# jdfxzzy/DPMN

Measured on AMD Instinct MI355X. Metric: SR images/sec (16x64->32x128, bs=48 per GPU, fp32 forward), higher is better.
Workload: dtype f32; 1 GPU; cfg1: TATT PSN + 3+3 PGRM (embed 96, windows 2/4/8) + CMM, forward-only; per_gpu_batch=48, global_batch=48, ranks=1, batches_in_flight=2, parallelism=dp1 (independent batch shards, no forward collective)

## Files before the change

dpmn_amd/csrc/common.h:

```cpp
#pragma once
#include <hip/hip_runtime.h>
#include <stdint.h>
#include "../../include/dpmn_hip.h"

typedef float f32x4 __attribute__((ext_vector_type(4)));

#define DPMN_CHECK_LAUNCH()                                                         \
  do {                                                                              \
    hipError_t e__ = hipGetLastError();                                             \
    if (e__ != hipSuccess) return dpmn_set_error(DPMN_ERR_LAUNCH, hipGetErrorString(e__)); \
  } while (0)

#define DPMN_REQUIRE(cond, msg)                                    \
  do {                                                             \
    if (!(cond)) return dpmn_set_error(DPMN_ERR_ARG, msg);         \
  } while (0)

int dpmn_set_error(int code, const char* msg);

__device__ __forceinline__ f32x4 mfma16(float a, float b, f32x4 c) {
  return __builtin_amdgcn_mfma_f32_16x16x4f32(a, b, c, 0, 0, 0);
}

__device__ __forceinline__ float erf_as(float x) {
// ... 97 lines not shown
    case 16: return xshfl<16>(v);
    case 32: return xshfl<32>(v);
    default: return __shfl_xor(v, o, 64);
  }
}
__device__ __forceinline__ float wave_sum(float v) {
#pragma unroll
  for (int o = 32; o > 0; o >>= 1) v += xshfl_v(v, o);
  return v;
}
__device__ __forceinline__ float wave_max(float v) {
#pragma unroll
  for (int o = 32; o > 0; o >>= 1) v = fmaxf(v, xshfl_v(v, o));
  return v;
}

constexpr unsigned long long DROP_PHI = 0x9E3779B97F4A7C15ull;
__device__ __forceinline__ unsigned long long drop_z0(unsigned long long seed, unsigned long long idx) { return idx * DROP_PHI + seed; }
__device__ __forceinline__ float drop_scale_z(unsigned long long z, float p, float inv_keep) {
  z ^= z >> 30; z *= 0xBF58476D1CE4E5B9ull;
  z ^= z >> 27; z *= 0x94D049BB133111EBull;
  z ^= z >> 31;
  const float u = (float)(unsigned)(z >> 40) * 5.9604644775390625e-8f;
  return u >= p ? inv_keep : 0.0f;
}
__device__ __forceinline__ float drop_scale(unsigned long long seed, unsigned long long idx, float p, float inv_keep) {
  return drop_scale_z(drop_z0(seed, idx), p, inv_keep);
}

static inline hipStream_t as_stream(dpmn_stream_t s) { return (hipStream_t)s; }

enum ProfTag { PT_CONV_IGEMM_128 = 0, PT_CONV_IGEMM_64, PT_CONV_IGEMM_NARROW, PT_CONV_SPLITK_REDUCE, PT_CONV_HALO, PT_CONV_HALO_C4,
               PT_GEMM_PW, PT_GEMM_WSTAT, PT_GEMM_KLOOP, PT_DWCONV_GELU, PT_WATTN8, PT_WATTN_SCALAR, PT_ATTN_FUSED, PT_BIGRU,
               PT_MHA32, PT_PATCH_EMBED, PT_SK_GATE, PT_TAIL, PT_DWPW_FUSED, PT_GEMM_WSTAT_LN, PT_CONV_IGEMM_SK, PT_ATTN_FUSED_BWD, PT_WATTN_BWD,
               PT_CONV_WGRAD, PT_GEMM_TN, PT_TN_REDUCE, PT_DWCONV_BWD, PT_WGRAD_UNPACK, PT_CONV_PACK, PT_AFFINE_ACT_BWD, PT_LN_BWD, PT_WATTN_MFMA32, PT_COUNT };
extern unsigned long long g_dpmn_prof_mask;
extern double g_dpmn_prof_hint_bytes;
extern int g_dpmn_bf16;
extern int g_dpmn_x3;
typedef __bf16 bf16x2 __attribute__((ext_vector_type(2)));
typedef __bf16 bf16x8 __attribute__((ext_vector_type(8)));
__device__ __forceinline__ uint2 pack_bf16x4(float a, float b, float c, float d) {
  typedef float f32x2_ __attribute__((ext_vector_type(2)));
  const bf16x2 lo = __builtin_convertvector((f32x2_){a, b}, bf16x2), hi = __builtin_convertvector((f32x2_){c, d}, bf16x2);
  return make_uint2(__builtin_bit_cast(unsigned, lo), __builtin_bit_cast(unsigned, hi));
}
__device__ __forceinline__ f32x4 mfma16_bf16(bf16x8 a, bf16x8 b, f32x4 c) {
  return __builtin_amdgcn_mfma_f32_16x16x32_bf16(a, b, c, 0, 0, 0);
}
__device__ __forceinline__ void x3_split2t(float a, float b, unsigned& h, unsigned& m, unsigned& l) {
  const unsigned ua = __float_as_uint(a), ub = __float_as_uint(b);
  h = __builtin_amdgcn_perm(ub, ua, 0x07060302u);
  const float ra = a - __uint_as_float(ua & 0xffff0000u), rb = b - __uint_as_float(ub & 0xffff0000u);
  const unsigned va = __float_as_uint(ra), vb = __float_as_uint(rb);
  m = __builtin_amdgcn_perm(vb, va, 0x07060302u);
  const float sa = ra - __uint_as_float(va & 0xffff0000u), sb = rb - __uint_as_float(vb & 0xffff0000u);
  l = __builtin_amdgcn_perm(__float_as_uint(sb), __float_as_uint(sa), 0x07060302u);
}
__device__ __forceinline__ void x3_split4t(const float4& v, uint2& h, uint2& m, uint2& l) {
  x3_split2t(v.x, v.y, h.x, m.x, l.x);
  x3_split2t(v.z, v.w, h.y, m.y, l.y);
}
struct ProfScope {
  int slot;
  hipStream_t st;
  ProfScope(int tag, hipStream_t s, double flops, double bytes);
  ~ProfScope();
// ... 15 lines not shown
```

dpmn_amd/csrc/pgrm.hip:

```cpp
#include "common.h"

namespace {

template <int C, int PATCH, bool FUSE>
__global__ __launch_bounds__(256) void k_patch_embed_ln(const float* __restrict__ img, int cin, const float* __restrict__ pf_w,
                                                         const float* __restrict__ pf_b, const float* __restrict__ pe_w,
                                                         const float* __restrict__ pe_b, const float* __restrict__ ln_w,
                                                         const float* __restrict__ ln_b, float* __restrict__ tok, int B,
                                                         int Hi, int Wi, float p_drop, unsigned long long seed) {
  constexpr int CQ = C / 4, KP = 3 * PATCH * PATCH;
  static_assert(!FUSE || PATCH == 2, "fused prior conv assumes 2x2 patches (one pixel per lane of the token quad)");
  __shared__ __attribute__((aligned(16))) float wt[KP * C];
  __shared__ float pfw[3 * 2 * 9 + 3];
  for (int i = threadIdx.x; i < KP * C; i += 256) wt[(i % KP) * C + i / KP] = pe_w[i];
  if (FUSE && threadIdx.x < 57) pfw[threadIdx.x] = threadIdx.x < 54 ? pf_w[threadIdx.x] : pf_b[threadIdx.x - 54];
  __syncthreads();
  const int Ht = Hi / PATCH, Wt = Wi / PATCH;
  const int lane = threadIdx.x & 63;
  long token = (long)blockIdx.x * 64 + (threadIdx.x >> 6) * 16 + (lane >> 2);
  const long ntok = (long)B * Ht * Wt;
  const bool valid = token < ntok;
  if (!valid) token = ntok - 1;
  const int part = lane & 3;
  const int b = token / (Ht * Wt), t = token % (Ht * Wt);
  const int th = t / Wt, tw = t % Wt;
  float in[KP];
  if (FUSE) {
    const int dy = part >> 1, dx = part & 1;
    const int y = th * 2 + dy, x = tw * 2 + dx;
    float a[3] = {pfw[54], pfw[55], pfw[56]};
#pragma unroll
    for (int ci = 0; ci < 2; ++ci)
#pragma unroll
      for (int ky = 0; ky < 3; ++ky) {
        const int yy = y + ky - 1;
#pragma unroll
        for (int kx = 0; kx < 3; ++kx) {
          const int xx = x + kx - 1;
          const bool inb = yy >= 0 && yy < Hi && xx >= 0 && xx < Wi;
          const float v = inb ? img[(((size_t)b * 2 + ci) * Hi + yy) * Wi + xx] : 0.f;
#pragma unroll
          for (int c = 0; c < 3; ++c) a[c] += pfw[((c * 2 + ci) * 3 + ky) * 3 + kx] * v;
        }
      }
    const int base = lane & ~3;
#pragma unroll
// ... 2 lines not shown
      for (int pix = 0; pix < 4; ++pix) in[c * 4 + pix] = __shfl(a[c], base + pix, 64);
  } else {
#pragma unroll
    for (int c = 0; c < 3; ++c)
#pragma unroll
      for (int dy = 0; dy < PATCH; ++dy)
#pragma unroll
        for (int dx = 0; dx < PATCH; ++dx)
          in[(c * PATCH + dy) * PATCH + dx] = img[(((size_t)b * cin + c) * Hi + th * PATCH + dy) * Wi + tw * PATCH + dx];
  }
  float o[CQ], s = 0.f;
#pragma unroll
  for (int i = 0; i < CQ; i += 4) {
    const float4 b4 = *reinterpret_cast<const float4*>(pe_b + part * CQ + i);
    o[i] = b4.x; o[i + 1] = b4.y; o[i + 2] = b4.z; o[i + 3] = b4.w;
  }
#pragma unroll
  for (int k = 0; k < KP; ++k) {
#pragma unroll
    for (int i = 0; i < CQ; i += 4) {
      const float4 w4 = *reinterpret_cast<const float4*>(wt + k * C + part * CQ + i);
      o[i] += w4.x * in[k]; o[i + 1] += w4.y * in[k]; o[i + 2] += w4.z * in[k]; o[i + 3] += w4.w * in[k];
    }
  }
#pragma unroll
  for (int i = 0; i < CQ; ++i) s += o[i];
  s += xshfl<1>(s); s += xshfl<2>(s);
  const float mean = s * (1.0f / C);
  float q = 0.f;
#pragma unroll
  for (int i = 0; i < CQ; ++i) { const float d = o[i] - mean; q += d * d; }
  q += xshfl<1>(q); q += xshfl<2>(q);
  const float rstd = 1.0f / sqrtf(q * (1.0f / C) + 1e-5f);
  if (!valid) return;
  float* dst = tok + (size_t)token * C + part * CQ;
  const float ik = p_drop > 0.f ? 1.0f / (1.0f - p_drop) : 1.f;
#pragma unroll
  for (int i = 0; i < CQ; i += 4) {
    const int c = part * CQ + i;
    float v[4] = {(o[i] - mean) * rstd * ln_w[c] + ln_b[c], (o[i + 1] - mean) * rstd * ln_w[c + 1] + ln_b[c + 1],
                  (o[i + 2] - mean) * rstd * ln_w[c + 2] + ln_b[c + 2], (o[i + 3] - mean) * rstd * ln_w[c + 3] + ln_b[c + 3]};
    if (p_drop > 0.f) {
      const unsigned long long z0 = drop_z0(seed, (unsigned long long)token * C + c);
#pragma unroll
      for (int r = 0; r < 4; ++r) v[r] *= drop_scale_z(z0 + (unsigned long long)r * DROP_PHI, p_drop, ik);
    }
    *reinterpret_cast<float4*>(dst + i) = make_float4(v[0], v[1], v[2], v[3]);
  }
}

template <int WS, int D, bool DROP>
__global__ __launch_bounds__(256) void k_window_attn(const float* __restrict__ q, const float* __restrict__ kv,
                                                      const float* __restrict__ bias_table, float* __restrict__ out, int B,
                                                      int H, int W, int C, int g, int shift, float p_drop,
                                                      unsigned long long seed) {
  constexpr int N = WS * WS;
  constexpr int CG = 2 * D;
  constexpr int QROWS = 64;
  constexpr int KROWS = 64;
  constexpr int LDR = CG + 4;
  constexpr int TBL = (2 * WS - 1) * (2 * WS - 1);
  extern __shared__ __attribute__((aligned(16))) float smem[];
  float* tbl = smem;
  float* base = smem + ((TBL * 2 + 3) & ~3);
  const int wave = threadIdx.x >> 6, lane = threadIdx.x & 63;
  const int slab_in_blk = wave >> 1, head = wave & 1;
  float* Qs = base + slab_in_blk * (QROWS + 2 * KROWS) * LDR;
  float* Ks = Qs + QROWS * LDR;
  float* Vs = Ks + KROWS * LDR;
  int* reg_s = reinterpret_cast<int*>(base + 2 * (QROWS + 2 * KROWS) * LDR) + slab_in_blk * KROWS;

  const int L = H * W;
  const int slabs_per_img = L / QROWS;
  const long slab = (long)blockIdx.x * 2 + slab_in_blk;
  const int b = slab / slabs_per_img;
  const int t0 = (slab % slabs_per_img) * QROWS;
  const int nWc = W / WS;
  const bool active = b < B;

  for (int i = threadIdx.x; i < TBL * 2; i += 256) tbl[i] = bias_table[i];
// ... 369 lines not shown
  constexpr int N = WS * WS, CG = 2 * D, LDR = CG + 4, TBL = (2 * WS - 1) * (2 * WS - 1), ROWS = WS == 16 ? 256 : 64, SETS = WS == 16 ? 1 : 2;
  const size_t smem = (size_t)(((TBL * 2 + 3) & ~3) + SETS * 2 * ROWS * LDR) * 4 + (size_t)SETS * ROWS * 4;
  static bool attr_set = false;
  if (!attr_set) {
    (void)hipFuncSetAttribute(reinterpret_cast<const void*>(&k_window_attn_mfma<WS, D, DROP>), hipFuncAttributeMaxDynamicSharedMemorySize, (int)smem);
    attr_set = true;
  }
  const long sets = (long)B * (H * W / ROWS);
  ProfScope prof(PT_WATTN_MFMA32, st, 4.0 * N * D * 2 * (double)B * H * W, 4.0 * 4 * CG * (double)B * H * W);
  hipLaunchKernelGGL((k_window_attn_mfma<WS, D, DROP>), dim3((unsigned)((sets + SETS - 1) / SETS)), dim3(WS == 16 ? 512 : 256), smem, st, q, kv, table,
                     out, B, H, W, C, g, shift, p_drop, seed);
  DPMN_CHECK_LAUNCH();
  return DPMN_OK;
}

template <int WS, int D, bool DROP>
int launch_window_attn(const float* q, const float* kv, const float* table, float* out, int B, int H, int W, int C, int g,
                       int shift, float p_drop, unsigned long long seed, hipStream_t st) {
  constexpr int N = WS * WS, CG = 2 * D, KROWS = 64, LDR = CG + 4, TBL = (2 * WS - 1) * (2 * WS - 1);
  const size_t smem = (size_t)(((TBL * 2 + 3) & ~3) + 2 * (64 + 2 * KROWS) * LDR) * 4 + 2 * KROWS * 4;
  static bool attr_set = false;
  if (!attr_set) {
    (void)hipFuncSetAttribute(reinterpret_cast<const void*>(&k_window_attn<WS, D, DROP>), hipFuncAttributeMaxDynamicSharedMemorySize, (int)smem);
    attr_set = true;
  }
  const long slabs = (long)B * (H * W / 64);
  ProfScope prof(PT_WATTN_SCALAR, st, 4.0 * N * D * 2 * (double)B * H * W, 4.0 * 4 * CG * (double)B * H * W);
  hipLaunchKernelGGL((k_window_attn<WS, D, DROP>), dim3((unsigned)((slabs + 1) / 2)), dim3(256), smem, st, q, kv, table, out, B, H, W,
                     C, g, shift, p_drop, seed);
  DPMN_CHECK_LAUNCH();
  return DPMN_OK;
}

__global__ void k_sk_gate(const float* __restrict__ partial, int parts_per_image, int L, const float* __restrict__ fc1_w,
                          const float* __restrict__ fc1_b, const float* __restrict__ fc2_w, const float* __restrict__ fc2_b,
                          float* __restrict__ attn_vec, int C, int G, int dmid) {
  extern __shared__ float sm[];
  float* S = sm;
  float* Z = sm + C;
  float* A = Z + dmid;
  const int b = blockIdx.x;
  for (int c = threadIdx.x; c < C; c += blockDim.x) {
    const float* pp = partial + (size_t)b * parts_per_image * C + c;
    float s0 = 0.f, s1 = 0.f, s2 = 0.f, s3 = 0.f;
    int p = 0;
    for (; p + 4 <= parts_per_image; p += 4) {
      s0 += pp[(size_t)p * C]; s1 += pp[(size_t)(p + 1) * C]; s2 += pp[(size_t)(p + 2) * C]; s3 += pp[(size_t)(p + 3) * C];
    }
    for (; p < parts_per_image; ++p) s0 += pp[(size_t)p * C];
    S[c] = ((s0 + s1) + (s2 + s3)) / (float)L;
  }
  __syncthreads();
  for (int j0 = 0; j0 < dmid; j0 += blockDim.x / 8) {
    const int j = j0 + threadIdx.x / 8, part = threadIdx.x & 7;
    float a = 0.f;
    if (j < dmid)
      for (int c = part; c < C; c += 8) a += fc1_w[j * C + c] * S[c];
    a += xshfl<1>(a); a += xshfl<2>(a); a += xshfl<4>(a);
    if (j < dmid && part == 0) Z[j] = gelu_erf(a + fc1_b[j]);
  }
  __syncthreads();
  for (int c = threadIdx.x; c < C; c += blockDim.x) {
    float a = fc2_b[c];
#pragma unroll 8
    for (int j = 0; j < dmid; ++j) a += fc2_w[c * dmid + j] * Z[j];
    A[c] = a;
  }
  __syncthreads();
  const int cg = C / G;
  for (int c = threadIdx.x; c < cg; c += blockDim.x) {
    float mx = -INFINITY;
    for (int g = 0; g < G; ++g) mx = fmaxf(mx, A[g * cg + c]);
    float den = 0.f;
    for (int g = 0; g < G; ++g) den += expf(A[g * cg + c] - mx);
    for (int g = 0; g < G; ++g) attn_vec[((size_t)b * G + g) * cg + c] = expf(A[g * cg + c] - mx) / den;
  }
}

template <bool R32>
__global__ __launch_bounds__(256) void k_dwconv_gelu(const float* __restrict__ y, const float* __restrict__ w,
                                                      const float* __restrict__ bias, float* __restrict__ g, int Ch, int r,
                                                      long planes, int apply_gelu, float* __restrict__ g2 = nullptr, int in_gelu = 0,
                                                      float p_drop = 0.f, unsigned long long seed = 0ull, int rb = 0) {
  const float inv_keep = p_drop > 0.f ? 1.0f / (1.0f - p_drop) : 1.0f;
  extern __shared__ __attribute__((aligned(16))) float sm[];
  const int wave = threadIdx.x >> 6, lane = threadIdx.x & 63;
  if (R32 || rb <= 0) rb = r;
  const int nb = r / rb;
  const long vplane = (long)blockIdx.x * 4 + wave;
  const long plane = R32 ? vplane : vplane / nb;
  const int y0 = R32 ? 0 : (int)(vplane % nb) * rb;
  const bool valid = plane < planes;
  const int c = valid ? (int)(plane % Ch) : 0;
  const int LD = r + 8, r4 = r >> 2;
  float* t = sm + wave * (rb + 2) * LD;
  if (valid) {
    const float* src = y + plane * r * r;
    float4 pre[R32 ? 4 : 1];
    if (R32) {
#pragma unroll
      for (int it = 0; it < 4; ++it) pre[it] = *reinterpret_cast<const float4*>(src + 4 * (lane + 64 * it));
    }
    const int nld = R32 ? 256 : (rb + 2) * r4;
#pragma unroll 4
    for (int it = 0; it < (R32 ? 4 : (nld + 63) / 64); ++it) {
      const int i = lane + 64 * it;
      if (!R32 && i >= nld) break;
      const int j = i / r4, x4 = (i - j * r4) * 4;
      const int yy = R32 ? j : y0 - 1 + j;
      float4 v = make_float4(0.f, 0.f, 0.f, 0.f);
      if (R32 || (yy >= 0 && yy < r)) {
        v = R32 ? pre[R32 ? it : 0] : *reinterpret_cast<const float4*>(src + yy * r + x4);
        if (in_gelu) { v.x = gelu_erf(v.x); v.y = gelu_erf(v.y); v.z = gelu_erf(v.z); v.w = gelu_erf(v.w); }
        if (p_drop > 0.f) {
          const unsigned long long e0 = (unsigned long long)(plane * r * r + yy * r + x4);
          const unsigned long long z0 = drop_z0(seed, e0);
          v.x *= drop_scale_z(z0, p_drop, inv_keep); v.y *= drop_scale_z(z0 + DROP_PHI, p_drop, inv_keep);
          v.z *= drop_scale_z(z0 + 2 * DROP_PHI, p_drop, inv_keep); v.w *= drop_scale_z(z0 + 3 * DROP_PHI, p_drop, inv_keep);
        }
      }
      *reinterpret_cast<float4*>(t + (R32 ? j + 1 : j) * LD + 4 + x4) = v;
    }
    if (R32)
      for (int i = lane; i < LD; i += 64) { t[i] = 0.f; t[(r + 1) * LD + i] = 0.f; }
    for (int i = lane; i < rb + 2; i += 64) { t[i * LD + 3] = 0.f; t[i * LD + 4 + r] = 0.f; }
  }
  __builtin_amdgcn_fence(__ATOMIC_ACQ_REL, "wavefront");
  if (!valid) return;
  float k[9];
#pragma unroll
  for (int i = 0; i < 9; ++i) k[i] = w[c * 9 + i];
  const float bv = bias[c];
  float* dst = g + plane * r * r + (size_t)y0 * r;
  for (int i = lane; i < rb * r4; i += 64) {
    const int yy = i / r4, x4 = (i - yy * r4) * 4;
    float a[4] = {bv, bv, bv, bv};
#pragma unroll
    for (int ky = 0; ky < 3; ++ky) {
      const float* p = t + (yy + ky) * LD + 4 + x4;
      const float4 m = *reinterpret_cast<const float4*>(p);
      const float l = p[-1], rr = p[4];
      const float k0 = k[ky * 3], k1 = k[ky * 3 + 1], k2 = k[ky * 3 + 2];
      a[0] += k0 * l + k1 * m.x + k2 * m.y;
      a[1] += k0 * m.x + k1 * m.y + k2 * m.z;
      a[2] += k0 * m.y + k1 * m.z + k2 * m.w;
      a[3] += k0 * m.z + k1 * m.w + k2 * rr;
    }
    if (apply_gelu == 2) {
      *reinterpret_cast<float4*>(dst + yy * r + x4) = make_float4(a[0], a[1], a[2], a[3]);
      *reinterpret_cast<float4*>(g2 + plane * r * r + (size_t)(y0 + yy) * r + x4) = make_float4(gelu_erf(a[0]), gelu_erf(a[1]), gelu_erf(a[2]), gelu_erf(a[3]));
      continue;
    }
    if (apply_gelu) {
#pragma unroll
      for (int q = 0; q < 4; ++q) a[q] = gelu_erf(a[q]);
    }
    *reinterpret_cast<float4*>(dst + yy * r + x4) = make_float4(a[0], a[1], a[2], a[3]);
  }
}

struct TailResid {
  const float* res[8];
  const float* wl[8];
  int n;
};
__global__ __launch_bounds__(256) void k_tail_conv2(const float* __restrict__ mid, const float* __restrict__ w,
                                                     const float* __restrict__ bias, const float* __restrict__ wl0, TailResid tr,
                                                     float* __restrict__ out, int B, int H, int W) {
  constexpr int Cm = 12;
  __shared__ __attribute__((aligned(16))) float ws[9 * Cm * Cm];
  for (int i = threadIdx.x; i < 9 * Cm * Cm; i += 256) {
    const int co = i % Cm, ci = (i / Cm) % Cm, tap = i / (Cm * Cm);
    ws[i] = w[(co * Cm + ci) * 9 + tap];
  }
  __syncthreads();
  const long pix = (long)blockIdx.x * 256 + threadIdx.x;
  if (pix >= (long)B * H * W) return;
  const int x = pix % W, y = (pix / W) % H, b = pix / ((long)W * H);
  float a[Cm];
#pragma unroll
  for (int co = 0; co < Cm; ++co) a[co] = bias[co];
#pragma unroll
  for (int ky = 0; ky < 3; ++ky) {
    const int yy = y + ky - 1;
    if (yy < 0 || yy >= H) continue;
#pragma unroll
    for (int kx = 0; kx < 3; ++kx) {
      const int xx = x + kx - 1;
      if (xx < 0 || xx >= W) continue;
      const float* src = mid + (((size_t)b * H + yy) * W + xx) * Cm;
      float v[Cm];
// ... 98 lines not shown
    if (ws == 8 && D == 16) {
      rc = p_drop > 0.f ? launch_window_attn8_mfma<true>(q, kv, bias_tables[g], out, B, H, W, C, g, sh, p_drop, seed, st)
                        : launch_window_attn8_mfma<false>(q, kv, bias_tables[g], out, B, H, W, C, g, sh, 0.f, 0ull, st);
      if (rc != DPMN_OK) return rc;
      continue;
    }
    if (D == 32 && (ws == 4 || ws == 8 || ws == 16)) {
      if (p_drop > 0.f)
        rc = ws == 4 ? launch_window_attn_mfma<4, 32, true>(q, kv, bias_tables[g], out, B, H, W, C, g, sh, st, p_drop, seed)
                     : (ws == 8 ? launch_window_attn_mfma<8, 32, true>(q, kv, bias_tables[g], out, B, H, W, C, g, sh, st, p_drop, seed)
                                : launch_window_attn_mfma<16, 32, true>(q, kv, bias_tables[g], out, B, H, W, C, g, sh, st, p_drop, seed));
      else
      rc = ws == 4 ? launch_window_attn_mfma<4, 32>(q, kv, bias_tables[g], out, B, H, W, C, g, sh, st)
                   : (ws == 8 ? launch_window_attn_mfma<8, 32>(q, kv, bias_tables[g], out, B, H, W, C, g, sh, st)
                              : launch_window_attn_mfma<16, 32>(q, kv, bias_tables[g], out, B, H, W, C, g, sh, st));
      if (rc != DPMN_OK) return rc;
      continue;
    }
#define WA_CASE(WSV, DV) if (ws == WSV && D == DV) rc = p_drop > 0.f \
      ? launch_window_attn<WSV, DV, true>(q, kv, bias_tables[g], out, B, H, W, C, g, sh, p_drop, seed, st) \
      : launch_window_attn<WSV, DV, false>(q, kv, bias_tables[g], out, B, H, W, C, g, sh, 0.f, 0ull, st); else
    WA_CASE(2, 16) WA_CASE(4, 16)
    return dpmn_set_error(DPMN_ERR_ARG, "window_attn: unsupported (window, head_dim); built: {2,4,8}x16, {4,8,16}x32");
#undef WA_CASE
    if (rc != DPMN_OK) return rc;
  }
  return DPMN_OK;
}

int dpmn_sk_gate_f32(const float* colsum_partials, int parts_per_image, int L, const float* fc1_w, const float* fc1_b,
                     const float* fc2_w, const float* fc2_b, float* attn_vec, int B, int C, int groups, int dmid,
                     dpmn_stream_t stream) {
  DPMN_REQUIRE(colsum_partials && fc1_w && fc1_b && fc2_w && fc2_b && attn_vec, "sk_gate: null pointer");
  hipLaunchKernelGGL(k_sk_gate, dim3(B), dim3(128), (size_t)(2 * C + dmid) * 4, as_stream(stream), colsum_partials,
                     parts_per_image, L, fc1_w, fc1_b, fc2_w, fc2_b, attn_vec, C, groups, dmid);
  DPMN_CHECK_LAUNCH();
  return DPMN_OK;
}

int dpmn_dwconv3x3_gelu_f32(const float* y, const float* w, const float* bias, float* g, int B, int Ch, int r,
                            dpmn_stream_t stream) {
  DPMN_REQUIRE(y && w && bias && g && r >= 4 && r <= 64 && r % 4 == 0, "dwconv: plane side must be a multiple of 4 in [4, 64]");
  const long planes = (long)B * Ch;
  const int rb = dwconv_band_rows(r);
  const long vplanes = planes * (r / rb);
  const size_t smem = (size_t)4 * (rb + 2) * (r + 8) * 4;
  if (smem > 48 * 1024) (void)hipFuncSetAttribute(reinterpret_cast<const void*>(&k_dwconv_gelu<false>), hipFuncAttributeMaxDynamicSharedMemorySize, (int)smem);
  ProfScope prof(PT_DWCONV_GELU, as_stream(stream), 18.0 * planes * r * r, 8.0 * planes * r * r);
  if (r == 32) hipLaunchKernelGGL(k_dwconv_gelu<true>, dim3((unsigned)((planes + 3) / 4)), dim3(256), smem, as_stream(stream), y, w, bias, g, Ch, r, planes, 1);
  else hipLaunchKernelGGL(k_dwconv_gelu<false>, dim3((unsigned)((vplanes + 3) / 4)), dim3(256), smem, as_stream(stream), y, w, bias, g, Ch, r, planes, 1,
                     static_cast<float*>(nullptr), 0, 0.f, 0ull, rb);
  DPMN_CHECK_LAUNCH();
  return DPMN_OK;
}

int dpmn_dwconv3x3_gelu_in_f32(const float* y, const float* w, const float* bias, float* g, int B, int Ch, int r, dpmn_stream_t stream) {
  DPMN_REQUIRE(y && w && bias && g && r >= 4 && r <= 64 && r % 4 == 0, "dwconv: plane side must be a multiple of 4 in [4, 64]");
  const long planes = (long)B * Ch;
  const int rb = dwconv_band_rows(r);
  const long vplanes = planes * (r / rb);
  const size_t smem = (size_t)4 * (rb + 2) * (r + 8) * 4;
  if (smem > 48 * 1024) (void)hipFuncSetAttribute(reinterpret_cast<const void*>(&k_dwconv_gelu<false>), hipFuncAttributeMaxDynamicSharedMemorySize, (int)smem);
  ProfScope prof(PT_DWCONV_GELU, as_stream(stream), 18.0 * planes * r * r, 8.0 * planes * r * r);
  if (r == 32) hipLaunchKernelGGL(k_dwconv_gelu<true>, dim3((unsigned)((planes + 3) / 4)), dim3(256), smem, as_stream(stream), y, w, bias, g, Ch, r, planes, 1,
                     static_cast<float*>(nullptr), 1, 0.f, 0ull);
  else hipLaunchKernelGGL(k_dwconv_gelu<false>, dim3((unsigned)((vplanes + 3) / 4)), dim3(256), smem, as_stream(stream), y, w, bias, g, Ch, r, planes, 1,
                     static_cast<float*>(nullptr), 1, 0.f, 0ull, rb);
  DPMN_CHECK_LAUNCH();
  return DPMN_OK;
}

int dpmn_dwconv3x3_f32(const float* y, const float* w, const float* bias, float* g, int B, int Ch, int r, dpmn_stream_t stream) {
  DPMN_REQUIRE(y && w && bias && g && r >= 4 && r <= 64 && r % 4 == 0, "dwconv: plane side must be a multiple of 4 in [4, 64]");
  const long planes = (long)B * Ch;
  const int rb = dwconv_band_rows(r);
  const long vplanes = planes * (r / rb);
  const size_t smem = (size_t)4 * (rb + 2) * (r + 8) * 4;
  if (smem > 48 * 1024) (void)hipFuncSetAttribute(reinterpret_cast<const void*>(&k_dwconv_gelu<false>), hipFuncAttributeMaxDynamicSharedMemorySize, (int)smem);
  if (r == 32) hipLaunchKernelGGL(k_dwconv_gelu<true>, dim3((unsigned)((planes + 3) / 4)), dim3(256), smem, as_stream(stream), y, w, bias, g, Ch, r, planes, 0);
  else hipLaunchKernelGGL(k_dwconv_gelu<false>, dim3((unsigned)((vplanes + 3) / 4)), dim3(256), smem, as_stream(stream), y, w, bias, g, Ch, r, planes, 0,
                     static_cast<float*>(nullptr), 0, 0.f, 0ull, rb);
  DPMN_CHECK_LAUNCH();
  return DPMN_OK;
}

int dpmn_dwconv3x3_train_f32(const float* y, const float* w, const float* bias, float* gpre, float* g, int in_gelu, float p_drop,
                             unsigned long long seed, int B, int Ch, int r, dpmn_stream_t stream) {
  DPMN_REQUIRE(y && w && bias && gpre && g && r >= 4 && r <= 64 && r % 4 == 0, "dwconv_train: plane side must be a multiple of 4 in [4, 64]");
  const long planes = (long)B * Ch;
  const int rb = dwconv_band_rows(r);
  const long vplanes = planes * (r / rb);
  const size_t smem = (size_t)4 * (rb + 2) * (r + 8) * 4;
  if (smem > 48 * 1024) (void)hipFuncSetAttribute(reinterpret_cast<const void*>(&k_dwconv_gelu<false>), hipFuncAttributeMaxDynamicSharedMemorySize, (int)smem);
  if (r == 32) hipLaunchKernelGGL(k_dwconv_gelu<true>, dim3((unsigned)((planes + 3) / 4)), dim3(256), smem, as_stream(stream), y, w, bias, gpre, Ch, r, planes, 2, g,
                     in_gelu, p_drop, seed);
  else hipLaunchKernelGGL(k_dwconv_gelu<false>, dim3((unsigned)((vplanes + 3) / 4)), dim3(256), smem, as_stream(stream), y, w, bias, gpre, Ch, r, planes, 2, g,
                     in_gelu, p_drop, seed, rb);
  DPMN_CHECK_LAUNCH();
  return DPMN_OK;
}

int dpmn_pgrm_tail_f32(const float* tokens, const float* w0, const float* b0, const float* w1, const float* b1,
                       const float* const* weight_list, const float* const* residuals, int n_residuals, float* mid_ws,
                       float* out, int B, int H, int W, int C, int hidden, int patch, dpmn_stream_t stream) {
  return dpmn_pgrm_tail_reuse_f32(tokens, w0, b0, w1, b1, weight_list, residuals, n_residuals, mid_ws, out, B, H, W, C, hidden, patch, 0, stream);
}

int dpmn_pgrm_tail_reuse_f32(const float* tokens, const float* w0, const float* b0, const float* w1, const float* b1,
                             const float* const* weight_list, const float* const* residuals, int n_residuals, float* mid_ws,
                             float* out, int B, int H, int W, int C, int hidden, int patch, int reuse_pack, dpmn_stream_t stream) {
  DPMN_REQUIRE(tokens && w0 && b0 && w1 && b1 && weight_list && mid_ws && out, "tail: null pointer");
  DPMN_REQUIRE(n_residuals >= 0 && n_residuals <= 8, "tail: at most 8 residuals");
  DPMN_REQUIRE(hidden == 3 && patch == 2 && C % 4 == 0, "tail: built for hidden_size=3, patch_size=2 (super_resolution.py:38-53)");
  const int Cm = hidden * patch * patch;
  const int Kp = ((9 * C + 31) / 32) * 32;
  float* wp = mid_ws + (size_t)B * H * W * Cm;
  if (!reuse_pack) {
    hipLaunchKernelGGL(k_pack_conv_w, dim3((Cm * Kp + 255) / 256), dim3(256), 0, as_stream(stream), w0, wp, Cm, C, 9, Kp);
    DPMN_CHECK_LAUNCH();
  }
  dpmn_conv_desc d{};
  d.in[0] = tokens; d.cseg[0] = C; d.B = B; d.Hin = H; d.Win = W;
  d.KH = 3; d.KW = 3; d.stride = 1; d.dil_y = 1; d.dil_x = 1; d.pad_y = 1; d.pad_x = 1;
  d.Hp = H; d.Wp = W; d.Hout = H; d.Wout = W; d.ostep = 1;
  d.w = wp; d.bias = b0; d.Cout = Cm; d.out = mid_ws;
  int rc = dpmn_conv2d_nhwc_f32(&d, stream);
  if (rc != DPMN_OK) return rc;
  TailResid tr{};
  tr.n = 0;
  for (int i = 1; i < n_residuals; ++i) {
    tr.res[tr.n] = residuals[i];
    tr.wl[tr.n] = weight_list[i];
// ... 11 lines not shown
```

dpmn_amd/csrc/runtime.hip:

```cpp
#include "common.h"
#include <string.h>
#include <stdlib.h>

static thread_local char g_err[512] = "";

int dpmn_set_error(int code, const char* msg) {
  strncpy(g_err, msg ? msg : "", sizeof(g_err) - 1);
  g_err[sizeof(g_err) - 1] = 0;
  return code;
}

unsigned long long g_dpmn_prof_mask = 0ull;
double g_dpmn_prof_hint_bytes = 0.0;
int g_dpmn_x3 = 0;
int g_dpmn_bf16 = 0;
namespace {
const char* const kTagNames[PT_COUNT] = {
    "k_conv_igemm<128,128>", "k_conv_igemm<64,64>", "k_conv_igemm<128,16|32>", "k_conv_splitk_reduce", "k_conv_halo", "k_conv_halo_c4",
    "k_gemm_pw", "k_gemm_wstat|rowreg", "k_gemm_kloop", "k_dwconv_gelu", "k_window_attn8_mfma", "k_window_attn<2|4>", "k_ln_qkv_window_attn",
    "k_bigru", "k_mha32", "k_patch_embed_ln", "k_sk_gate", "k_tail_conv2", "k_mlp_dw_pw", "k_gemm_wstat|rowreg<LN prologue>", "k_conv_igemm_sk", "k_ln_qkv_window_attn_bwd", "k_window_attn_bwd_mfma",
    "k_conv_wgrad", "k_gemm_tn_reg", "k_tn_reduce_multi", "k_dwconv_bwd", "k_wgrad_unpack_multi", "k_conv_pack_multi", "k_affine_act_bwd", "k_ln_bwd", "k_window_attn_mfma<4|8|16,32>"};
struct Rec { int tag; double flops, bytes; };
struct Prof {
  int cap = 0, count = 0, limit = 0;
  hipEvent_t* ev = nullptr;
  Rec* rec = nullptr;
} g_prof;
}

int dpmn_prof_open(int tag, hipStream_t st, double flops, double bytes) {
  if (g_prof.count >= g_prof.limit) return -1;
  const int i = g_prof.count++;
  g_prof.rec[i] = Rec{tag, flops, bytes};
  (void)hipEventRecord(g_prof.ev[2 * i], st);
  return i;
}
void dpmn_prof_close(int slot, hipStream_t st) { (void)hipEventRecord(g_prof.ev[2 * slot + 1], st); }

extern "C" {
int dpmn_abi_version(void) { return 5; }
int dpmn_set_compute_dtype(int mode) {
  DPMN_REQUIRE(mode >= 0 && mode <= 2, "set_compute_dtype: 0 = f32, 1 = bf16 operands, 2 = f32 via three bf16 terms");
  g_dpmn_bf16 = mode == 1;
  g_dpmn_x3 = mode == 2;
  return DPMN_OK;
}
int dpmn_get_compute_dtype(void) { return g_dpmn_x3 ? 2 : g_dpmn_bf16; }
const char* dpmn_last_error(void) { return g_err; }

int dpmn_profile_tag_count(void) { return PT_COUNT; }
int dpmn_profile_hint_bytes(double bytes) { g_dpmn_prof_hint_bytes = bytes; return DPMN_OK; }
const char* dpmn_profile_tag_name(int tag) { return tag >= 0 && tag < PT_COUNT ? kTagNames[tag] : ""; }

// ... 37 lines not shown
```

Measured before the change: 6373 images/s.

## Stage patch-embed stores, preload SK gate weights, persistent r32 dwconv kernel

After: 6491 images/s, median of 6. 1.8% higher.

```diff
diff --git a/dpmn_amd/csrc/common.h b/dpmn_amd/csrc/common.h
--- a/dpmn_amd/csrc/common.h
+++ b/dpmn_amd/csrc/common.h
@@ -153,7 +153,7 @@
 
 enum ProfTag { PT_CONV_IGEMM_128 = 0, PT_CONV_IGEMM_64, PT_CONV_IGEMM_NARROW, PT_CONV_SPLITK_REDUCE, PT_CONV_HALO, PT_CONV_HALO_C4,
                PT_GEMM_PW, PT_GEMM_WSTAT, PT_GEMM_KLOOP, PT_DWCONV_GELU, PT_WATTN8, PT_WATTN_SCALAR, PT_ATTN_FUSED, PT_BIGRU,
-               PT_MHA32, PT_PATCH_EMBED, PT_SK_GATE, PT_TAIL, PT_DWPW_FUSED, PT_GEMM_WSTAT_LN, PT_CONV_IGEMM_SK, PT_ATTN_FUSED_BWD, PT_WATTN_BWD,
+               PT_MHA32, PT_PATCH_EMBED, PT_SK_GATE, PT_TAIL, PT_GEMM_WSTAT_LN, PT_CONV_IGEMM_SK, PT_ATTN_FUSED_BWD, PT_WATTN_BWD,
                PT_CONV_WGRAD, PT_GEMM_TN, PT_TN_REDUCE, PT_DWCONV_BWD, PT_WGRAD_UNPACK, PT_CONV_PACK, PT_AFFINE_ACT_BWD, PT_LN_BWD, PT_WATTN_MFMA32, PT_COUNT };
 extern unsigned long long g_dpmn_prof_mask;
 extern double g_dpmn_prof_hint_bytes;
diff --git a/dpmn_amd/csrc/pgrm.hip b/dpmn_amd/csrc/pgrm.hip
--- a/dpmn_amd/csrc/pgrm.hip
+++ b/dpmn_amd/csrc/pgrm.hip
@@ -1,4 +1,5 @@
 #include "common.h"
+#include <atomic>
 
 namespace {
 
@@ -12,6 +13,8 @@
   static_assert(!FUSE || PATCH == 2, "fused prior conv assumes 2x2 patches (one pixel per lane of the token quad)");
   __shared__ __attribute__((aligned(16))) float wt[KP * C];
   __shared__ float pfw[3 * 2 * 9 + 3];
+  constexpr int LDT = C + 4;
+  __shared__ __attribute__((aligned(16))) float stg[4 * 16 * LDT];
   for (int i = threadIdx.x; i < KP * C; i += 256) wt[(i % KP) * C + i / KP] = pe_w[i];
   if (FUSE && threadIdx.x < 57) pfw[threadIdx.x] = threadIdx.x < 54 ? pf_w[threadIdx.x] : pf_b[threadIdx.x - 54];
   __syncthreads();
@@ -80,8 +83,8 @@
   for (int i = 0; i < CQ; ++i) { const float d = o[i] - mean; q += d * d; }
   q += xshfl<1>(q); q += xshfl<2>(q);
   const float rstd = 1.0f / sqrtf(q * (1.0f / C) + 1e-5f);
-  if (!valid) return;
-  float* dst = tok + (size_t)token * C + part * CQ;
+  const int wave = threadIdx.x >> 6;
+  float* sw = stg + wave * 16 * LDT;
   const float ik = p_drop > 0.f ? 1.0f / (1.0f - p_drop) : 1.f;
 #pragma unroll
   for (int i = 0; i < CQ; i += 4) {
@@ -93,7 +96,18 @@
 #pragma unroll
       for (int r = 0; r < 4; ++r) v[r] *= drop_scale_z(z0 + (unsigned long long)r * DROP_PHI, p_drop, ik);
     }
-    *reinterpret_cast<float4*>(dst + i) = make_float4(v[0], v[1], v[2], v[3]);
+    *reinterpret_cast<float4*>(sw + (lane >> 2) * LDT + c) = make_float4(v[0], v[1], v[2], v[3]);
+  }
+  __builtin_amdgcn_fence(__ATOMIC_ACQ_REL, "wavefront");
+  const long tok0 = (long)blockIdx.x * 64 + wave * 16;
+  const long left = ntok - tok0;
+  const int nfl = (left >= 16 ? 16 : (left > 0 ? (int)left : 0)) * C;
+  float* dst = tok + (size_t)tok0 * C;
+#pragma unroll
+  for (int it = 0; it < C / 16; ++it) {
+    const int idx = (it * 64 + lane) * 4;
+    const int row = idx / C, col = idx - row * C;
+    if (idx < nfl) *reinterpret_cast<float4*>(dst + idx) = *reinterpret_cast<const float4*>(sw + row * LDT + col);
   }
 }
 
@@ -529,43 +543,72 @@
   return DPMN_OK;
 }
 
-__global__ void k_sk_gate(const float* __restrict__ partial, int parts_per_image, int L, const float* __restrict__ fc1_w,
+constexpr int SKG_T = 512, SKG_STAGE = 12;
+__global__ __launch_bounds__(SKG_T) void k_sk_gate(const float* __restrict__ partial, int parts_per_image, int L, const float* __restrict__ fc1_w,
                           const float* __restrict__ fc1_b, const float* __restrict__ fc2_w, const float* __restrict__ fc2_b,
                           float* __restrict__ attn_vec, int C, int G, int dmid) {
   extern __shared__ float sm[];
   float* S = sm;
   float* Z = sm + C;
   float* A = Z + dmid;
-  const int b = blockIdx.x;
-  for (int c = threadIdx.x; c < C; c += blockDim.x) {
-    const float* pp = partial + (size_t)b * parts_per_image * C + c;
-    float s0 = 0.f, s1 = 0.f, s2 = 0.f, s3 = 0.f;
-    int p = 0;
-    for (; p + 4 <= parts_per_image; p += 4) {
-      s0 += pp[(size_t)p * C]; s1 += pp[(size_t)(p + 1) * C]; s2 += pp[(size_t)(p + 2) * C]; s3 += pp[(size_t)(p + 3) * C];
-    }
-    for (; p < parts_per_image; ++p) s0 += pp[(size_t)p * C];
-    S[c] = ((s0 + s1) + (s2 + s3)) / (float)L;
+  float* Q = A + C;
+  float* W1 = Q + 4 * C;
+  const int nw = dmid * C;
+  float* W2 = W1 + nw;
+  float* B1 = W2 + nw;
+  float* B2 = B1 + dmid;
+  const int b = blockIdx.x, tid = threadIdx.x;
+  if (tid < SKG_T / 2) {
+    const int p4 = parts_per_image & ~3;
+    for (int i = tid; i < 4 * C; i += SKG_T / 2) {
+      const int q = i / C, c = i - q * C;
+      const float* pp = partial + (size_t)b * parts_per_image * C + c;
+      float s = 0.f;
+#pragma unroll 8
+      for (int p = q; p < p4; p += 4) s += pp[(size_t)p * C];
+      if (q == 0)
+        for (int p = p4; p < parts_per_image; ++p) s += pp[(size_t)p * C];
+      Q[i] = s;
+    }
+  } else {
+    const int n = 2 * nw + dmid + C, t = tid - SKG_T / 2;
+    for (int i0 = t; i0 < n; i0 += SKG_STAGE * (SKG_T / 2)) {
+      float v[SKG_STAGE];
+#pragma unroll
+      for (int u = 0; u < SKG_STAGE; ++u) {
+        int i = i0 + u * (SKG_T / 2);
+        i = i < n ? i : n - 1;
+        const float* src = i < nw ? fc1_w + i : (i < 2 * nw ? fc2_w + (i - nw) : (i < 2 * nw + dmid ? fc1_b + (i - 2 * nw) : fc2_b + (i - 2 * nw - dmid)));
+        v[u] = *src;
+      }
+#pragma unroll
+      for (int u = 0; u < SKG_STAGE; ++u) {
+        const int i = i0 + u * (SKG_T / 2);
+        if (i < n) W1[i] = v[u];
+      }
+    }
   }
   __syncthreads();
-  for (int j0 = 0; j0 < dmid; j0 += blockDim.x / 8) {
-    const int j = j0 + threadIdx.x / 8, part = threadIdx.x & 7;
+  for (int c = tid; c < C; c += SKG_T) S[c] = ((Q[c] + Q[C + c]) + (Q[2 * C + c] + Q[3 * C + c])) / (float)L;
+  __syncthreads();
+  for (int j0 = 0; j0 < dmid; j0 += SKG_T / 8) {
+    const int j = j0 + tid / 8, part = tid & 7;
     float a = 0.f;
     if (j < dmid)
-      for (int c = part; c < C; c += 8) a += fc1_w[j * C + c] * S[c];
+      for (int c = part; c < C; c += 8) a += W1[j * C + c] * S[c];
     a += xshfl<1>(a); a += xshfl<2>(a); a += xshfl<4>(a);
-    if (j < dmid && part == 0) Z[j] = gelu_erf(a + fc1_b[j]);
+    if (j < dmid && part == 0) Z[j] = gelu_erf(a + B1[j]);
   }
   __syncthreads();
-  for (int c = threadIdx.x; c < C; c += blockDim.x) {
-    float a = fc2_b[c];
+  for (int c = tid; c < C; c += SKG_T) {
+    float a = B2[c];
 #pragma unroll 8
-    for (int j = 0; j < dmid; ++j) a += fc2_w[c * dmid + j] * Z[j];
+    for (int j = 0; j < dmid; ++j) a += W2[c * dmid + j] * Z[j];
     A[c] = a;
   }
   __syncthreads();
   const int cg = C / G;
-  for (int c = threadIdx.x; c < cg; c += blockDim.x) {
+  for (int c = tid; c < cg; c += SKG_T) {
     float mx = -INFINITY;
     for (int g = 0; g < G; ++g) mx = fmaxf(mx, A[g * cg + c]);
     float den = 0.f;
@@ -574,40 +617,34 @@
   }
 }
 
-template <bool R32>
 __global__ __launch_bounds__(256) void k_dwconv_gelu(const float* __restrict__ y, const float* __restrict__ w,
                                                       const float* __restrict__ bias, float* __restrict__ g, int Ch, int r,
-                                                      long planes, int apply_gelu, float* __restrict__ g2 = nullptr, int in_gelu = 0,
-                                                      float p_drop = 0.f, unsigned long long seed = 0ull, int rb = 0) {
+                                                      long planes, int apply_gelu, float* __restrict__ g2, int in_gelu,
+                                                      float p_drop, unsigned long long seed, int rb) {
   const float inv_keep = p_drop > 0.f ? 1.0f / (1.0f - p_drop) : 1.0f;
   extern __shared__ __attribute__((aligned(16))) float sm[];
   const int wave = threadIdx.x >> 6, lane = threadIdx.x & 63;
-  if (R32 || rb <= 0) rb = r;
+  if (rb <= 0) rb = r;
   const int nb = r / rb;
   const long vplane = (long)blockIdx.x * 4 + wave;
-  const long plane = R32 ? vplane : vplane / nb;
-  const int y0 = R32 ? 0 : (int)(vplane % nb) * rb;
+  const long plane = vplane / nb;
+  const int y0 = (int)(vplane % nb) * rb;
   const bool valid = plane < planes;
   const int c = valid ? (int)(plane % Ch) : 0;
   const int LD = r + 8, r4 = r >> 2;
   float* t = sm + wave * (rb + 2) * LD;
   if (valid) {
     const float* src = y + plane * r * r;
-    float4 pre[R32 ? 4 : 1];
-    if (R32) {
-#pragma unroll
-      for (int it = 0; it < 4; ++it) pre[it] = *reinterpret_cast<const float4*>(src + 4 * (lane + 64 * it));
-    }
-    const int nld = R32 ? 256 : (rb + 2) * r4;
+    const int nld = (rb + 2) * r4;
 #pragma unroll 4
-    for (int it = 0; it < (R32 ? 4 : (nld + 63) / 64); ++it) {
+    for (int it = 0; it < (nld + 63) / 64; ++it) {
       const int i = lane + 64 * it;
-      if (!R32 && i >= nld) break;
+      if (i >= nld) break;
       const int j = i / r4, x4 = (i - j * r4) * 4;
-      const int yy = R32 ? j : y0 - 1 + j;
+      const int yy = y0 - 1 + j;
       float4 v = make_float4(0.f, 0.f, 0.f, 0.f);
-      if (R32 || (yy >= 0 && yy < r)) {
-        v = R32 ? pre[R32 ? it : 0] : *reinterpret_cast<const float4*>(src + yy * r + x4);
+      if (yy >= 0 && yy < r) {
+        v = *reinterpret_cast<const float4*>(src + yy * r + x4);
         if (in_gelu) { v.x = gelu_erf(v.x); v.y = gelu_erf(v.y); v.z = gelu_erf(v.z); v.w = gelu_erf(v.w); }
         if (p_drop > 0.f) {
           const unsigned long long e0 = (unsigned long long)(plane * r * r + yy * r + x4);
@@ -616,10 +653,8 @@
           v.z *= drop_scale_z(z0 + 2 * DROP_PHI, p_drop, inv_keep); v.w *= drop_scale_z(z0 + 3 * DROP_PHI, p_drop, inv_keep);
         }
       }
-      *reinterpret_cast<float4*>(t + (R32 ? j + 1 : j) * LD + 4 + x4) = v;
-    }
-    if (R32)
-      for (int i = lane; i < LD; i += 64) { t[i] = 0.f; t[(r + 1) * LD + i] = 0.f; }
+      *reinterpret_cast<float4*>(t + j * LD + 4 + x4) = v;
+    }
     for (int i = lane; i < rb + 2; i += 64) { t[i * LD + 3] = 0.f; t[i * LD + 4 + r] = 0.f; }
   }
   __builtin_amdgcn_fence(__ATOMIC_ACQ_REL, "wavefront");
@@ -654,6 +689,89 @@
     }
     *reinterpret_cast<float4*>(dst + yy * r + x4) = make_float4(a[0], a[1], a[2], a[3]);
   }
+}
+
+template <int MODE, bool MORE>
+__device__ __forceinline__ void dwconv32_plane(float* __restrict__ t, float4 (&pre)[4], const float* __restrict__ y, const float* __restrict__ w,
+                                               const float* __restrict__ bias, float* __restrict__ g, float* __restrict__ g2, int Ch,
+                                               int plane, int next, int lane, int in_gelu, float p_drop, float inv_keep,
+                                               unsigned long long seed) {
+  constexpr int LD = 40;
+  const int c = plane % Ch;
+  float k[9];
+#pragma unroll
+  for (int i = 0; i < 9; ++i) k[i] = w[c * 9 + i];
+  const float bv = bias[c];
+#pragma unroll
+  for (int it = 0; it < 4; ++it) {
+    const int i = lane + 64 * it;
+    const int j = i >> 3, x4 = (i & 7) * 4;
+    float4 v = pre[it];
+    if (in_gelu) { v.x = gelu_erf(v.x); v.y = gelu_erf(v.y); v.z = gelu_erf(v.z); v.w = gelu_erf(v.w); }
+    if (p_drop > 0.f) {
+      const unsigned long long z0 = drop_z0(seed, (unsigned long long)plane * 1024 + 4 * i);
+      v.x *= drop_scale_z(z0, p_drop, inv_keep); v.y *= drop_scale_z(z0 + DROP_PHI, p_drop, inv_keep);
+      v.z *= drop_scale_z(z0 + 2 * DROP_PHI, p_drop, inv_keep); v.w *= drop_scale_z(z0 + 3 * DROP_PHI, p_drop, inv_keep);
+    }
+    *reinterpret_cast<float4*>(t + (j + 1) * LD + 4 + x4) = v;
+  }
+  if (MORE) {
+    const float* src = y + (size_t)next * 1024;
+#pragma unroll
+    for (int it = 0; it < 4; ++it) pre[it] = *reinterpret_cast<const float4*>(src + 4 * (lane + 64 * it));
+  }
+  __builtin_amdgcn_fence(__ATOMIC_ACQ_REL, "wavefront");
+  float* dst = g + (size_t)plane * 1024;
+#pragma unroll
+  for (int it = 0; it < 4; ++it) {
+    const int i = lane + 64 * it;
+    const int yy = i >> 3, x4 = (i & 7) * 4;
+    float a[4] = {bv, bv, bv, bv};
+#pragma unroll
+    for (int ky = 0; ky < 3; ++ky) {
+      const float* p = t + (yy + ky) * LD + 4 + x4;
+      const float4 m = *reinterpret_cast<const float4*>(p);
+      const float l = p[-1], rr = p[4];
+      const float k0 = k[ky * 3], k1 = k[ky * 3 + 1], k2 = k[ky * 3 + 2];
+      a[0] += k0 * l + k1 * m.x + k2 * m.y;
+      a[1] += k0 * m.x + k1 * m.y + k2 * m.z;
+      a[2] += k0 * m.y + k1 * m.z + k2 * m.w;
+      a[3] += k0 * m.z + k1 * m.w + k2 * rr;
+    }
+    if (MODE == 2) {
+      *reinterpret_cast<float4*>(dst + 4 * i) = make_float4(a[0], a[1], a[2], a[3]);
+      *reinterpret_cast<float4*>(g2 + (size_t)plane * 1024 + 4 * i) = make_float4(gelu_erf(a[0]), gelu_erf(a[1]), gelu_erf(a[2]), gelu_erf(a[3]));
+    } else {
+      if (MODE == 1) {
+#pragma unroll
+        for (int q = 0; q < 4; ++q) a[q] = gelu_erf(a[q]);
+      }
+      *reinterpret_cast<float4*>(dst + 4 * i) = make_float4(a[0], a[1], a[2], a[3]);
+    }
+  }
+  __builtin_amdgcn_fence(__ATOMIC_ACQ_REL, "wavefront");
+}
+
+template <int MODE>
+__global__ __launch_bounds__(256) void k_dwconv_gelu_r32(const float* __restrict__ y, const float* __restrict__ w,
+                                                          const float* __restrict__ bias, float* __restrict__ g, float* __restrict__ g2,
+                                                          int Ch, int planes, int in_gelu, float p_drop, unsigned long long seed) {
+  constexpr int LD = 40;
+  __shared__ __attribute__((aligned(16))) float sm[4 * 34 * LD];
+  const int wave = __builtin_amdgcn_readfirstlane((int)(threadIdx.x >> 6)), lane = threadIdx.x & 63;
+  const float inv_keep = p_drop > 0.f ? 1.0f / (1.0f - p_drop) : 1.0f;
+  const int nw = (int)gridDim.x * 4;
+  int plane = (int)blockIdx.x * 4 + wave;
+  if (plane >= planes) return;
+  float* t = sm + wave * 34 * LD;
+  for (int i = lane; i < LD; i += 64) { t[i] = 0.f; t[33 * LD + i] = 0.f; }
+  if (lane < 34) { t[lane * LD + 3] = 0.f; t[lane * LD + 36] = 0.f; }
+  float4 pre[4];
+#pragma unroll
+  for (int it = 0; it < 4; ++it) pre[it] = *reinterpret_cast<const float4*>(y + (size_t)plane * 1024 + 4 * (lane + 64 * it));
+  for (int next = plane + nw; next < planes; plane = next, next += nw)
+    dwconv32_plane<MODE, true>(t, pre, y, w, bias, g, g2, Ch, plane, next, lane, in_gelu, p_drop, inv_keep, seed);
+  dwconv32_plane<MODE, false>(t, pre, y, w, bias, g, g2, Ch, plane, plane, lane, in_gelu, p_drop, inv_keep, seed);
 }
 
 struct TailResid {
@@ -818,72 +936,76 @@
                      const float* fc2_w, const float* fc2_b, float* attn_vec, int B, int C, int groups, int dmid,
                      dpmn_stream_t stream) {
   DPMN_REQUIRE(colsum_partials && fc1_w && fc1_b && fc2_w && fc2_b && attn_vec, "sk_gate: null pointer");
-  hipLaunchKernelGGL(k_sk_gate, dim3(B), dim3(128), (size_t)(2 * C + dmid) * 4, as_stream(stream), colsum_partials,
+  DPMN_REQUIRE(B >= 1 && parts_per_image >= 1 && L >= 1 && C >= 1 && dmid >= 1 && groups >= 1 && C % groups == 0, "sk_gate: bad shape");
+  const size_t smem = ((size_t)7 * C + 2 * dmid + (size_t)2 * dmid * C) * 4;
+  DPMN_REQUIRE(smem <= 160 * 1024, "sk_gate: fc1 / fc2 do not fit in LDS");
+  if (smem > 48 * 1024) (void)hipFuncSetAttribute(reinterpret_cast<const void*>(&k_sk_gate), hipFuncAttributeMaxDynamicSharedMemorySize, (int)smem);
+  hipLaunchKernelGGL(k_sk_gate, dim3(B), dim3(SKG_T), smem, as_stream(stream), colsum_partials,
                      parts_per_image, L, fc1_w, fc1_b, fc2_w, fc2_b, attn_vec, C, groups, dmid);
   DPMN_CHECK_LAUNCH();
   return DPMN_OK;
 }
 
+static unsigned dwconv32_grid(long planes) {
+  static std::atomic<int> cus[64];
+  int dev = 0;
+  if (hipGetDevice(&dev) != hipSuccess || dev < 0 || dev >= 64) dev = 0;
+  int n_cu = cus[dev].load(std::memory_order_relaxed);
+  if (n_cu < 1) {
+    if (hipDeviceGetAttribute(&n_cu, hipDeviceAttributeMultiprocessorCount, dev) != hipSuccess || n_cu < 1) n_cu = 256;
+    cus[dev].store(n_cu, std::memory_order_relaxed);
+  }
+  const long cap = 7L * n_cu * 4;
+  const long per = (planes + cap - 1) / cap;
+  const long waves = (planes + per - 1) / per;
+  return (unsigned)((waves + 3) / 4);
+}
+
+static int launch_dwconv(const float* y, const float* w, const float* bias, float* g, float* g2, int apply_gelu, int in_gelu, float p_drop,
+                         unsigned long long seed, int B, int Ch, int r, hipStream_t st) {
+  const long planes = (long)B * Ch;
+  DPMN_REQUIRE(planes >= 1 && planes <= (1L << 30), "dwconv: B * Ch out of range");
+  if (r == 32) {
+    const dim3 grid(dwconv32_grid(planes));
+#define DW32(MODE) hipLaunchKernelGGL(k_dwconv_gelu_r32<MODE>, grid, dim3(256), 0, st, y, w, bias, g, g2, Ch, (int)planes, in_gelu, p_drop, seed)
+    if (apply_gelu == 2) DW32(2);
+    else if (apply_gelu == 1) DW32(1);
+    else DW32(0);
+#undef DW32
+  } else {
+    const int rb = dwconv_band_rows(r);
+    const long vplanes = planes * (r / rb);
+    const size_t smem = (size_t)4 * (rb + 2) * (r + 8) * 4;
+    if (smem > 48 * 1024) (void)hipFuncSetAttribute(reinterpret_cast<const void*>(&k_dwconv_gelu), hipFuncAttributeMaxDynamicSharedMemorySize, (int)smem);
+    hipLaunchKernelGGL(k_dwconv_gelu, dim3((unsigned)((vplanes + 3) / 4)), dim3(256), smem, st, y, w, bias, g, Ch, r, planes, apply_gelu, g2,
+                       in_gelu, p_drop, seed, rb);
+  }
+  DPMN_CHECK_LAUNCH();
+  return DPMN_OK;
+}
+
 int dpmn_dwconv3x3_gelu_f32(const float* y, const float* w, const float* bias, float* g, int B, int Ch, int r,
                             dpmn_stream_t stream) {
   DPMN_REQUIRE(y && w && bias && g && r >= 4 && r <= 64 && r % 4 == 0, "dwconv: plane side must be a multiple of 4 in [4, 64]");
-  const long planes = (long)B * Ch;
-  const int rb = dwconv_band_rows(r);
-  const long vplanes = planes * (r / rb);
-  const size_t smem = (size_t)4 * (rb + 2) * (r + 8) * 4;
-  if (smem > 48 * 1024) (void)hipFuncSetAttribute(reinterpret_cast<const void*>(&k_dwconv_gelu<false>), hipFuncAttributeMaxDynamicSharedMemorySize, (int)smem);
-  ProfScope prof(PT_DWCONV_GELU, as_stream(stream), 18.0 * planes * r * r, 8.0 * planes * r * r);
-  if (r == 32) hipLaunchKernelGGL(k_dwconv_gelu<true>, dim3((unsigned)((planes + 3) / 4)), dim3(256), smem, as_stream(stream), y, w, bias, g, Ch, r, planes, 1);
-  else hipLaunchKernelGGL(k_dwconv_gelu<false>, dim3((unsigned)((vplanes + 3) / 4)), dim3(256), smem, as_stream(stream), y, w, bias, g, Ch, r, planes, 1,
-                     static_cast<float*>(nullptr), 0, 0.f, 0ull, rb);
-  DPMN_CHECK_LAUNCH();
-  return DPMN_OK;
+  ProfScope prof(PT_DWCONV_GELU, as_stream(stream), 18.0 * B * Ch * r * r, 8.0 * B * Ch * r * r);
+  return launch_dwconv(y, w, bias, g, nullptr, 1, 0, 0.f, 0ull, B, Ch, r, as_stream(stream));
 }
 
 int dpmn_dwconv3x3_gelu_in_f32(const float* y, const float* w, const float* bias, float* g, int B, int Ch, int r, dpmn_stream_t stream) {
   DPMN_REQUIRE(y && w && bias && g && r >= 4 && r <= 64 && r % 4 == 0, "dwconv: plane side must be a multiple of 4 in [4, 64]");
-  const long planes = (long)B * Ch;
-  const int rb = dwconv_band_rows(r);
-  const long vplanes = planes * (r / rb);
-  const size_t smem = (size_t)4 * (rb + 2) * (r + 8) * 4;
-  if (smem > 48 * 1024) (void)hipFuncSetAttribute(reinterpret_cast<const void*>(&k_dwconv_gelu<false>), hipFuncAttributeMaxDynamicSharedMemorySize, (int)smem);
-  ProfScope prof(PT_DWCONV_GELU, as_stream(stream), 18.0 * planes * r * r, 8.0 * planes * r * r);
-  if (r == 32) hipLaunchKernelGGL(k_dwconv_gelu<true>, dim3((unsigned)((planes + 3) / 4)), dim3(256), smem, as_stream(stream), y, w, bias, g, Ch, r, planes, 1,
-                     static_cast<float*>(nullptr), 1, 0.f, 0ull);
-  else hipLaunchKernelGGL(k_dwconv_gelu<false>, dim3((unsigned)((vplanes + 3) / 4)), dim3(256), smem, as_stream(stream), y, w, bias, g, Ch, r, planes, 1,
-                     static_cast<float*>(nullptr), 1, 0.f, 0ull, rb);
-  DPMN_CHECK_LAUNCH();
-  return DPMN_OK;
+  ProfScope prof(PT_DWCONV_GELU, as_stream(stream), 18.0 * B * Ch * r * r, 8.0 * B * Ch * r * r);
+  return launch_dwconv(y, w, bias, g, nullptr, 1, 1, 0.f, 0ull, B, Ch, r, as_stream(stream));
 }
 
 int dpmn_dwconv3x3_f32(const float* y, const float* w, const float* bias, float* g, int B, int Ch, int r, dpmn_stream_t stream) {
   DPMN_REQUIRE(y && w && bias && g && r >= 4 && r <= 64 && r % 4 == 0, "dwconv: plane side must be a multiple of 4 in [4, 64]");
-  const long planes = (long)B * Ch;
-  const int rb = dwconv_band_rows(r);
-  const long vplanes = planes * (r / rb);
-  const size_t smem = (size_t)4 * (rb + 2) * (r + 8) * 4;
-  if (smem > 48 * 1024) (void)hipFuncSetAttribute(reinterpret_cast<const void*>(&k_dwconv_gelu<false>), hipFuncAttributeMaxDynamicSharedMemorySize, (int)smem);
-  if (r == 32) hipLaunchKernelGGL(k_dwconv_gelu<true>, dim3((unsigned)((planes + 3) / 4)), dim3(256), smem, as_stream(stream), y, w, bias, g, Ch, r, planes, 0);
-  else hipLaunchKernelGGL(k_dwconv_gelu<false>, dim3((unsigned)((vplanes + 3) / 4)), dim3(256), smem, as_stream(stream), y, w, bias, g, Ch, r, planes, 0,
-                     static_cast<float*>(nullptr), 0, 0.f, 0ull, rb);
-  DPMN_CHECK_LAUNCH();
-  return DPMN_OK;
+  return launch_dwconv(y, w, bias, g, nullptr, 0, 0, 0.f, 0ull, B, Ch, r, as_stream(stream));
 }
 
 int dpmn_dwconv3x3_train_f32(const float* y, const float* w, const float* bias, float* gpre, float* g, int in_gelu, float p_drop,
                              unsigned long long seed, int B, int Ch, int r, dpmn_stream_t stream) {
   DPMN_REQUIRE(y && w && bias && gpre && g && r >= 4 && r <= 64 && r % 4 == 0, "dwconv_train: plane side must be a multiple of 4 in [4, 64]");
-  const long planes = (long)B * Ch;
-  const int rb = dwconv_band_rows(r);
-  const long vplanes = planes * (r / rb);
-  const size_t smem = (size_t)4 * (rb + 2) * (r + 8) * 4;
-  if (smem > 48 * 1024) (void)hipFuncSetAttribute(reinterpret_cast<const void*>(&k_dwconv_gelu<false>), hipFuncAttributeMaxDynamicSharedMemorySize, (int)smem);
-  if (r == 32) hipLaunchKernelGGL(k_dwconv_gelu<true>, dim3((unsigned)((planes + 3) / 4)), dim3(256), smem, as_stream(stream), y, w, bias, gpre, Ch, r, planes, 2, g,
-                     in_gelu, p_drop, seed);
-  else hipLaunchKernelGGL(k_dwconv_gelu<false>, dim3((unsigned)((vplanes + 3) / 4)), dim3(256), smem, as_stream(stream), y, w, bias, gpre, Ch, r, planes, 2, g,
-                     in_gelu, p_drop, seed, rb);
-  DPMN_CHECK_LAUNCH();
-  return DPMN_OK;
+  return launch_dwconv(y, w, bias, gpre, g, 2, in_gelu, p_drop, seed, B, Ch, r, as_stream(stream));
 }
 
 int dpmn_pgrm_tail_f32(const float* tokens, const float* w0, const float* b0, const float* w1, const float* b1,
diff --git a/dpmn_amd/csrc/runtime.hip b/dpmn_amd/csrc/runtime.hip
--- a/dpmn_amd/csrc/runtime.hip
+++ b/dpmn_amd/csrc/runtime.hip
@@ -18,7 +18,7 @@
 const char* const kTagNames[PT_COUNT] = {
     "k_conv_igemm<128,128>", "k_conv_igemm<64,64>", "k_conv_igemm<128,16|32>", "k_conv_splitk_reduce", "k_conv_halo", "k_conv_halo_c4",
     "k_gemm_pw", "k_gemm_wstat|rowreg", "k_gemm_kloop", "k_dwconv_gelu", "k_window_attn8_mfma", "k_window_attn<2|4>", "k_ln_qkv_window_attn",
-    "k_bigru", "k_mha32", "k_patch_embed_ln", "k_sk_gate", "k_tail_conv2", "k_mlp_dw_pw", "k_gemm_wstat|rowreg<LN prologue>", "k_conv_igemm_sk", "k_ln_qkv_window_attn_bwd", "k_window_attn_bwd_mfma",
+    "k_bigru", "k_mha32", "k_patch_embed_ln", "k_sk_gate", "k_tail_conv2", "k_gemm_wstat|rowreg<LN prologue>", "k_conv_igemm_sk", "k_ln_qkv_window_attn_bwd", "k_window_attn_bwd_mfma",
     "k_conv_wgrad", "k_gemm_tn_reg", "k_tn_reduce_multi", "k_dwconv_bwd", "k_wgrad_unpack_multi", "k_conv_pack_multi", "k_affine_act_bwd", "k_ln_bwd", "k_window_attn_mfma<4|8|16,32>"};
 struct Rec { int tag; double flops, bytes; };
 struct Prof {
```
